# furkanyesiler/acoss

Hardware: AMD Instinct MI355X
Metric: track-pairs/sec on N x N Serra09 Qmax (HPCP, T=2000) (higher is better)
Workload: dtype f32

## Files before the change

### acoss_amd/_lib.py

```python
import ctypes
import os

import numpy as np

_HERE = os.path.dirname(os.path.abspath(__file__))
LIB_PATH = os.environ.get("ACX_LIB") or os.path.join(_HERE, "csrc", "libacx.so")

ACX_OK = 0
ACX_ERR_INVALID = -1
ACX_ERR_HIP = -2
ACX_ERR_NOMEM = -3
ACX_ERR_STATE = -4
ACX_ERR_SHORT = -5
ACX_ERR_UNSUPPORTED = -6

EXPORTS = [
    "acx_abi_version", "acx_create", "acx_destroy", "acx_last_error", "acx_set_scratch_limit",
    "acx_upload_pool", "acx_serra09_default_params", "acx_serra09_pairs", "acx_serra09_debug_pair",
    "acx_serra09_embed_len", "acx_profile_enable", "acx_profile_reset", "acx_profile_count",
    "acx_profile_get", "acx_debug_sqrt", "acx_debug_ef_sqrt", "acx_upload_pool_f64", "acx_simple_pairs",
    "acx_ef_upload_pool", "acx_earlyfusion_pairs", "acx_ef_debug_pair", "acx_sw_binary",
    "acx_chenfusion_pairs", "acx_csm_binary_sw", "acx_upload_raw_pool", "acx_download_pool",
    "acx_simple_upload_raw_pool", "acx_download_pool_f64", "acx_snf_fuse", "acx_qmax_binary",
    "acx_ef_block_features", "acx_ef_upload_raw_pool", "acx_snf_fuse_dists", "acx_grid_plan", "acx_pool_lengths", "acx_grid_run", "acx_grid_scatter", "acx_pair_grid",
    "acx_set_nonfinite_policy", "acx_nonfinite_zeroed", "acx_ef_pool_begin", "acx_ef_pool_tracks", "acx_ef_pool_end",
    "acx_set_ef_gemm", "acx_hip_versions",
    "acx_dev_alloc", "acx_dev_free", "acx_dev_read", "acx_dev_sync",
    "acx_comm_id", "acx_comm_init", "acx_comm_destroy", "acx_grid_allgather", "acx_pair_grid_ranks", "acx_set_ef_fuse",
    "acx_device_info", "acx_ef_debug_pairs",
    "acx_ftm2d_default_params", "acx_ftm2d_pool_begin", "acx_ftm2d_pool_tracks", "acx_ftm2d_pool_end",
    "acx_ftm2d_upload_shingles", "acx_ftm2d_download_shingles", "acx_ftm2d_debug_track", "acx_ftm2d_pairs",
    "acx_rank_columns", "acx_topk_rows",
    "acx_query_scores", "acx_query_topk", "acx_query_ranks", "acx_query_topk_lists",
    "acx_serra09_debug_bits", "acx_serra09_plan", "acx_serra09_family_name",
    "acx_pool_append", "acx_pool_append_raw", "acx_pool_append_f64", "acx_ef_pool_append", "acx_ftm2d_append_shingles",
    "acx_pool_truncate",
    "acx_serra09_align", "acx_qmax_locate_binary",
    "acx_serra09_align_paths", "acx_qmax_path_binary",
]
ABI_VERSION = 4
COMM_ID_BYTES = 128

ALGO_SERRA09, ALGO_CHENFUSION, ALGO_SIMPLE, ALGO_EARLYFUSION, ALGO_FTM2D = 0, 1, 2, 3, 4
GRID_PLANES = {ALGO_SERRA09: 1, ALGO_CHENFUSION: 2, ALGO_SIMPLE: 1, ALGO_EARLYFUSION: 4, ALGO_FTM2D: 1}


class AcxError(RuntimeError):
    """A libacx call failed (HIP error, missing device, out of device memory ...)."""

# ... 130 lines not shown
    L.acx_set_nonfinite_policy.argtypes = [vp, ctypes.c_int32]
    L.acx_nonfinite_zeroed.restype = ctypes.c_int64
    L.acx_nonfinite_zeroed.argtypes = [vp]
    L.acx_upload_pool.argtypes = [vp, fp, lp, ctypes.c_int32, ctypes.c_int32]
    L.acx_upload_raw_pool.argtypes = [vp, fp, lp, ctypes.c_int32, ctypes.c_int32, ctypes.c_int32, lp]
    L.acx_download_pool.argtypes = [vp, fp, ctypes.c_int64]
    L.acx_serra09_default_params.restype = None
    L.acx_serra09_default_params.argtypes = [pp]
    L.acx_serra09_pairs.argtypes = [vp, ip, ctypes.c_int64, pp, fp]
    L.acx_chenfusion_pairs.argtypes = [vp, ip, ctypes.c_int64, pp, fp]
    L.acx_serra09_debug_pair.argtypes = [vp, ctypes.c_int32, ctypes.c_int32, pp, fp, fp, fp, fp, fp, ip, fp, ip]
    L.acx_serra09_debug_bits.argtypes = [vp, ip, ctypes.c_int64, pp, fp, ctypes.POINTER(ctypes.c_uint8), ctypes.POINTER(ctypes.c_int64)]
    L.acx_serra09_plan.argtypes = [lp, ctypes.c_int32, ip, ctypes.c_int64, pp, ctypes.c_int64, ctypes.POINTER(Serra09PlanRec)]
    L.acx_serra09_family_name.restype = ctypes.c_char_p
    L.acx_serra09_family_name.argtypes = [ctypes.c_int32, ctypes.c_int32]
    L.acx_serra09_embed_len.restype = ctypes.c_int32
    L.acx_serra09_embed_len.argtypes = [ctypes.c_int32, pp]
    L.acx_profile_enable.argtypes = [vp, ctypes.c_int]
    L.acx_profile_reset.argtypes = [vp]
    L.acx_profile_count.argtypes = [vp]
    L.acx_profile_get.argtypes = [vp, ctypes.c_int, ctypes.c_char_p, ctypes.c_int,
                                  ctypes.POINTER(ctypes.c_double), lp, lp]
    L.acx_debug_sqrt.argtypes = [vp, fp, ctypes.c_int64, fp]
    L.acx_debug_ef_sqrt.argtypes = [vp, fp, ctypes.c_int64, fp]
    dp = ctypes.POINTER(ctypes.c_double)
    L.acx_upload_pool_f64.argtypes = [vp, dp, lp, ctypes.c_int32, ctypes.c_int32]
    L.acx_simple_upload_raw_pool.argtypes = [vp, fp, lp, ctypes.c_int32, ctypes.c_int32, ctypes.c_int32, ctypes.c_int32,
                                             ctypes.c_int32, lp]
    L.acx_download_pool_f64.argtypes = [vp, dp, ctypes.c_int64]
    L.acx_simple_pairs.argtypes = [vp, ip, ctypes.c_int64, ctypes.c_int32, ctypes.c_int32, dp]
# ... 144 lines not shown
def serra09_plan(lengths, pairs, params=None, scratch_limit=0):
    L = load()
    lengths = np.ascontiguousarray(lengths, dtype=np.int64)
    pairs = np.ascontiguousarray(pairs, dtype=np.int32).reshape(-1, 2)
    params = params if params is not None else serra09_params()
    out = np.zeros(len(pairs), dtype=np.dtype(Serra09PlanRec))
    rc = L.acx_serra09_plan(_lptr(lengths), len(lengths), _iptr(pairs), len(pairs), ctypes.byref(params), int(scratch_limit),
                            out.ctypes.data_as(ctypes.POINTER(Serra09PlanRec)))
    if rc != ACX_OK:
        err = AcxError("acx_serra09_plan: code %d: %s" % (rc, (L.acx_last_error(None) or b"bad argument").decode()))
        err.code = rc
        raise err
    return out


def serra09_family_name(family, m):
    name = load().acx_serra09_family_name(int(family), int(m))
    if name is None:
        raise ValueError("unknown Serra09 kernel family %r" % (family,))
    return name.decode()


def grid_scatter(lengths, spec, gathered, rank_stride, planes, mirror, first=0, count=-1):
    L = load()
    lengths = np.ascontiguousarray(lengths, dtype=np.int64)
    gathered = np.ascontiguousarray(gathered, dtype=np.float32)
    n = len(lengths)
    for P in planes:
        if P.dtype != np.float32 or P.shape != (n, n) or not P.flags["C_CONTIGUOUS"]:
            raise ValueError("grid_scatter: planes must be C-contiguous (N, N) float32")
# ... 726 lines not shown
```

### acoss_amd/csrc/acx.hip

```cpp
#include <hip/hip_runtime.h>

#include <chrono>
#include <dlfcn.h>
#include <rccl/rccl.h>

#include <algorithm>
#include <cmath>
#include <cstdio>
#include <cstdlib>
#include <cstring>
#include <string>
#include <vector>

#include "../../include/acx.h"
#include "serra09_kernels.hpp"
#include "serra09_long_kernels.hpp"
#include "serra09_locate_kernels.hpp"
#include "serra09_path_kernels.hpp"
#include "prep_kernels.hpp"
#include "snf_kernels.hpp"
#include "simple_kernels.hpp"
#include "ef_kernels.hpp"
#include "ef_rowstat2_kernels.hpp"
#include "ef_gemm_dma_kernels.hpp"
// ... 271 lines not shown
{
    if (p.m < 1 || p.m > acx::MAX_M_LONG) return fail(c, ACX_ERR_UNSUPPORTED, "serra09: m must be in 1..33 on the device");
    if (p.tau < 1) return fail(c, ACX_ERR_INVALID, "serra09: tau must be >= 1");
    if (!(p.kappa >= 0.0f && p.kappa <= 1.0f)) return fail(c, ACX_ERR_INVALID, "serra09: kappa must be in [0, 1]");
    if (p.dp_start != 2 && p.dp_start != 3) return fail(c, ACX_ERR_INVALID, "serra09: dp_start must be 2 or 3");
    if (p.pct_mode < 0 || p.pct_mode > 3) return fail(c, ACX_ERR_INVALID, "serra09: pct_mode must be 0..3");
    if (p.oti_target != 0 && p.oti_target != 1) return fail(c, ACX_ERR_INVALID, "serra09: oti_target must be 0 or 1");
    if (!(p.gamma_o >= 0.0f) || !(p.gamma_e >= 0.0f)) return fail(c, ACX_ERR_INVALID, "serra09: gammas must be >= 0");
    if (p.arith != ACX_ARITH_EXACT && p.arith != ACX_ARITH_F16X2) return fail(c, ACX_ERR_INVALID, "serra09: arith must be ACX_ARITH_EXACT or ACX_ARITH_F16X2");
    if (p.arith == ACX_ARITH_F16X2 && p.m != 9) return fail(c, ACX_ERR_UNSUPPORTED, "serra09: the f16x2 Gram exists for the default stack size m = 9 only");
    return ACX_OK;
}

constexpr int64_t POOL_SLACK = 96;

bool launch_band(acx_ctx *c, int m, const PairDesc *dpd, int B, int maxRows, int cls, const acx_serra09_params &p, int role, int write_d2,
                 int want_eps)
{
    const float *operands = p.arith == ACX_ARITH_F16X2 ? reinterpret_cast<const float *>(c->d_fh + POOL_SLACK * acx::FH) : c->d_frot + POOL_SLACK * acx::FROT;
    acx::BandLaunch L{c->stream, operands, c->active_toff(), c->d_normtab + POOL_SLACK, c->d_noff, c->d_scratch, c->d_thr,
                      c->d_bits, p.kappa, p.pct_mode, p.inclusive, p.oti_target};
    return acx::launch_band_kernel(L, m, dpd, B, maxRows, acx::serra09_band_family(cls, m, p.arith), role, write_d2, want_eps, p.arith);
}

template <int M>
void launch_normtab(acx_ctx *c, int maxM, int span, int first, int count)
{
    hipLaunchKernelGGL((acx::normtab_kernel<M>), dim3(count, (maxM + 255) / 256, acx::NBIN), dim3(256), 0, c->stream,
                       c->active_frames(), c->active_toff() + first, c->d_noff + first, c->d_normtab + POOL_SLACK, span);
}

#ifdef ACX_FAST_BUILD
#ifndef ACX_FAST_BUILD_M
#define ACX_FAST_BUILD_M 9
#endif
#define ACX_M_SWITCH(m_, CALL) switch (m_) { case ACX_FAST_BUILD_M: CALL(ACX_FAST_BUILD_M); break; default: handled = false; }
#else
// ... 477 lines not shown
        }
        int64_t cls_cells[NC + 1];
        for (int cl = 0; cl <= NC; ++cl) {
            cls_cells[cl] = 0;
            const int b0 = cls_begin[cl], Bc = cls_begin[cl + 1] - b0;
            if (Bc <= 0) continue;
            const acx::Serra09Extent ce = acx::serra09_extent(pd, b0, b0 + Bc);
            cls_cells[cl] = ce.cells;
            if (cl < NC) {
                bool ok = true;
                for (int cq = 0; cq < NC; ++cq) {
                    const int q0 = key_begin[NC * cl + cq], Bq = key_begin[NC * cl + cq + 1] - q0;
                    if (Bq <= 0) continue;
                    const acx::Serra09Extent qe = acx::serra09_extent(pd, q0, q0 + Bq);
                    ProfScope ps(c, KS_BAND, qe.cells);
                    ok = ok && launch_band(c, p.m, S.d_pd + q0, Bq, qe.Mr, cq, p, 1, 0, dbg ? 1 : 0);
                }
                if (!bits_free) { ACX_HIP(c, hipStreamWaitEvent(c->stream, Sprev.done, 0)); bits_free = true; }
                {
                    ProfScope ps(c, KS_BAND, ce.cells);
                    ok = ok && launch_band(c, p.m, S.d_pd + b0, Bc, ce.Mq, cl, p, 0, dbg ? 1 : 0, dbg ? 1 : 0);
                }
                if (use_q) ACX_HIP(c, hipEventRecord(S.cls_ev[cl], c->stream));
                if (!ok) return fail(c, ACX_ERR_UNSUPPORTED, "serra09: this build of libacx has no band kernel for the requested m");
            } else {
                if (!bits_free) { ACX_HIP(c, hipStreamWaitEvent(c->stream, Sprev.done, 0)); bits_free = true; }
                launch_streaming_class(c, S.d_pd + b0, &pd[b0], Bc, ce, p);
            }
        }
        {
            hipError_t wait_err = hipSuccess;
            auto sweep = [&](bool dmax, float *dst, hipStream_t qs) {
                for (int cl = 0; cl <= NC; ++cl) {
                    const int b0 = cls_begin[cl], Bc = cls_begin[cl + 1] - b0;
                    if (Bc <= 0) continue;
                    if (use_q) { const hipError_t e_ = hipStreamWaitEvent(qs, S.cls_ev[cl], 0); if (e_ != hipSuccess) wait_err = e_; }
// ... 2823 lines not shown
                r.Mq = pd[k2].Mq; r.Mr = pd[k2].Mr;
                r.batch = batch;
                r.cr = cl; r.cq = band ? acx::serra09_row_class(pd[k2].Mq) : acx::SERRA09_NC;
                r.row_family = band ? acx::serra09_band_family(r.cr, params->m, params->arith) : ACX_SERRA09_FAMILY_STREAMING;
                r.col_family = band ? acx::serra09_band_family(r.cq, params->m, params->arith) : ACX_SERRA09_FAMILY_STREAMING;
                r.sweep_cols = sw.cols; r.sweep_pack = sw.pack;
            }
        }
        k0 = k;
    }
    return ACX_OK;
}

const char *acx_serra09_family_name(int32_t family, int32_t m) { return acx::serra09_family_name(family, m); }

int acx_pool_lengths(acx_ctx *c, int32_t algo, int64_t *lengths, int32_t capacity, int32_t *n_tracks)
{
    if (!c) return ACX_ERR_INVALID;
    std::vector<int64_t> len;
    const int rc = pool_lengths(c, algo, len);
    if (rc != ACX_OK) return rc;
    if (n_tracks) *n_tracks = (int32_t)len.size();
    if (lengths) {
        if (capacity < (int32_t)len.size()) return fail(c, ACX_ERR_INVALID, "pool_lengths: buffer too small");
        std::copy(len.begin(), len.end(), lengths);
    }
    return ACX_OK;
}

static const std::vector<acx_grid_tile> &cached_plan(acx_ctx *c, const std::vector<int64_t> &len, const acx_grid_spec &spec)
// ... 996 lines not shown
```

### acoss_amd/csrc/acx_band.hip

```cpp
#include <hip/hip_runtime.h>

#include "serra09_kernels.hpp"
#include "serra09_band2_kernels.hpp"
#include "serra09_plan.hpp"

namespace acx {

namespace {

template <int M>
bool launch_band_m(const BandLaunch &L, const PairDesc *dpd, int B, int maxRows, int family, int role, int write_d2, int want_eps, int arith)
{
    const dim3 grid((maxRows + BAND - 1) / BAND, B, 1);
#define ACX_BAND_K(V4_, R_, W_, A_) hipLaunchKernelGGL((band_kernel<M, V4_, R_, W_, A_>), grid, dim3(BAND_THREADS), 0, L.stream, \
                                                  L.frot, L.toff, L.normtab, L.noff, dpd, L.scratch, L.thr, L.bits, L.kappa, \
                                                  L.pct_mode, L.inclusive, L.oti_target, want_eps)
#define ACX_BAND_A(V4_, A_) do { if (role) ACX_BAND_K(V4_, 1, false, A_); else if (write_d2) ACX_BAND_K(V4_, 0, true, A_); else ACX_BAND_K(V4_, 0, false, A_); } while (0)
#define ACX_BAND(V4_) do { if (arith == ACX_ARITH_EXACT) ACX_BAND_A(V4_, 0); else if constexpr (M == 9) ACX_BAND_A(V4_, 1); else return false; return true; } while (0)
#define ACX_BAND2_K(R_, W_, NV_, GL_) hipLaunchKernelGGL((band2_kernel<M, R_, W_, NV_, GL_>), grid, dim3(64 * B2Geom<NV_, GL_>::WAVES), 0, L.stream, L.frot, L.normtab, \
                                                         dpd, L.scratch, L.thr, L.bits, L.pct_mode, L.inclusive, L.oti_target, want_eps)
#define ACX_BAND2(NV_, GL_) do { if constexpr (M <= 9) { if (arith != ACX_ARITH_EXACT) return false; \
                                     if (role) ACX_BAND2_K(1, false, NV_, GL_); else if (write_d2) ACX_BAND2_K(0, true, NV_, GL_); else ACX_BAND2_K(0, false, NV_, GL_); \
                                     return true; } return false; } while (0)
    if (arith != ACX_ARITH_EXACT && arith != ACX_ARITH_F16X2) return false;
    switch (family) {
    case ACX_SERRA09_FAMILY_BAND2_4ROWS: ACX_BAND2(B2_NV, 16);
    case ACX_SERRA09_FAMILY_BAND2_2ROWS: ACX_BAND2(B2_NV, 32);
    case ACX_SERRA09_FAMILY_BAND2_MID: ACX_BAND2(B2_NV_MID, 32);
    case ACX_SERRA09_FAMILY_BAND_2: ACX_BAND(2);
    case ACX_SERRA09_FAMILY_BAND_4: ACX_BAND(4);
    case ACX_SERRA09_FAMILY_BAND_8: ACX_BAND(8);
    }
// ... 13 lines not shown
#define ACX_CASE(M_) case M_: return launch_band_m<M_>(L, dpd, B, maxRows, family, role, write_d2, want_eps, arith);
#ifdef ACX_FAST_BUILD
#ifndef ACX_FAST_BUILD_M
#define ACX_FAST_BUILD_M 9
#endif
        ACX_CASE(ACX_FAST_BUILD_M)
#else
        ACX_CASE(1) ACX_CASE(2) ACX_CASE(3) ACX_CASE(4) ACX_CASE(5) ACX_CASE(6) ACX_CASE(7) ACX_CASE(8)
        ACX_CASE(9) ACX_CASE(10) ACX_CASE(11) ACX_CASE(12) ACX_CASE(13) ACX_CASE(14) ACX_CASE(15) ACX_CASE(16)
#endif
#undef ACX_CASE
    }
    return false;
}


}

#ifdef ACX_TIMING
extern "C" int acx_dev_band_timing(unsigned long long *out, int reset)
{
    if (hipDeviceSynchronize() != hipSuccess) return -1;
    if (hipMemcpyFromSymbol(out, HIP_SYMBOL(acx::g_band_clk), sizeof(unsigned long long) * 32) != hipSuccess) return -1;
    if (reset) {
        unsigned long long z[32] = {0};
        if (hipMemcpyToSymbol(HIP_SYMBOL(acx::g_band_clk), z, sizeof(z)) != hipSuccess) return -1;
    }
    return 0;
}
#endif
// ... 1 lines not shown
```

### acoss_amd/csrc/serra09_kernels.hpp

```cpp
#pragma once
#include <hip/hip_runtime.h>
#include <stdint.h>
#include <type_traits>

namespace acx {

constexpr int NBIN = 12;
constexpr int SEL_BINS = 2048;
constexpr int MAX_M = 16;
constexpr int NGUARD = 80;

struct PctPos { float kf, fl, ce; int32_t ilo, ihi, k; };
__host__ __device__ inline PctPos pct_position(int n, float kappa, int pct_mode)
{
    PctPos p;
    p.kf = (n > 1) ? (float)(n - 1) * kappa : (float)n * kappa;
    p.fl = floorf(p.kf); p.ce = ceilf(p.kf);
    int ilo = (int)p.fl, ihi = (int)p.ce;
    ilo = ilo < 0 ? 0 : (ilo > n - 1 ? n - 1 : ilo);
    ihi = ihi < 0 ? 0 : (ihi > n - 1 ? n - 1 : ihi);
    int k = ilo;
    if (pct_mode == 3) {
        k = (int)floorf(p.kf + 0.5f);
        k = k > n - 1 ? n - 1 : k;
// ... 747 lines not shown
    if (e >= n) return;
    const int t = e / NBIN, b = e - t * NBIN;
    out[o0 * NBIN + e] = in[(toff_in[track] + (int64_t)t * tau) * NBIN + b];
}

struct BandLaunch {
    hipStream_t stream;
    const float *frot;
    const int64_t *toff;
    const float *normtab;
    const int64_t *noff;
    float *scratch, *thr;
    unsigned long long *bits;
    float kappa;
    int pct_mode, inclusive, oti_target;
};
bool launch_band_kernel(const BandLaunch &L, int m, const struct PairDesc *dpd, int B, int maxRows, int family, int role,
                        int write_d2, int want_eps, int arith);

#ifdef ACX_ABL
#define ACX_ABL_EXIT(n_, val_) do { if (ACX_ABL == (n_)) { if ((val_) == 1.2345e-30f) thr[0] = 1.0f; return; } } while (0)
#else
#define ACX_ABL_EXIT(n_, val_) do { } while (0)
#endif

#ifdef ACX_TIMING
__device__ unsigned long long g_band_clk[32];
struct StampT { unsigned long long t; int base; };
#define ACX_STAMP(slot) do { const unsigned long long now_ = __builtin_readcyclecounter(); \
        if (lane == 0) atomicAdd(&g_band_clk[tstamp_.base + (slot)], now_ - tstamp_.t); tstamp_.t = now_; } while (0)
#else
#define ACX_STAMP(slot) do { } while (0)
#endif
// ... 36 lines not shown
    static constexpr bool HIST_IN_ROW = ROWP >= 64 + 2 * FBINS;
    static constexpr int PBINS = NV >= 32 ? 512 : 256;
    static constexpr int PGRP = NV >= 32 ? 1 : 2;
    static constexpr float PDELTA = NV >= 32 ? 0.04f : (NV >= 16 ? 0.15f : 0.0f);
    static constexpr int GBINS = 32 * NV;
    static constexpr int TAIL_FLOATS = BAND * ROWP + (HIST_IN_ROW ? 0 : 8 * FBINS);
    static_assert(SelGeom<GBINS>::SLOTS + 64 + 4 <= ROWP, "generic selection must fit the wave's own exchange row");
    static_assert(HIST_IN_ROW || (BAND * ROWP) % FBINS == 0, "fast histograms must be aligned to their size");
    static_assert(NV == 8 || NV == 16 || NV == 32, "row owners hold 8, 16 or 32 consecutive slots");
    __device__ static __forceinline__ int hist_off(int wave)
    {
        return HIST_IN_ROW ? ((wave * ROWP + 64 + FBINS - 1) & ~(FBINS - 1)) : BAND * ROWP + wave * FBINS;
    }
};

template <int NV, int ROLE, bool TC_VIA_LDS, typename TCG>
__device__ __forceinline__ void band_row_bits(const float (&xr)[NV], const TCG (&tcg)[NV / 4], float thr_row, float *myrow, int lane,
                                              int row, int MB, int cshift, const PairDesc &P, float *__restrict__ thr,
                                              unsigned long long *__restrict__ bits)
{
    using RG = RowGeom<NV>;
    constexpr int CH = NV / 4;
    typedef float f32x4_u __attribute__((ext_vector_type(4), aligned(4)));
    float *X = thr + P.offX;
    if (ROLE == 0 && bits) {
        float tcv[NV];
        if constexpr (TC_VIA_LDS) {
            float *tr = myrow + 4 * lane + 4 * ((4 * lane) / NV);
#pragma unroll
            for (int q = 0; q < CH; ++q) *reinterpret_cast<float4 *>(tr + q * (256 + 4 * (256 / NV))) = make_float4(tcg[q].x, tcg[q].y, tcg[q].z, tcg[q].w);
            wave_lds_fence();
            const float *mine = myrow + lane * RG::LNP;
#pragma unroll
            for (int j = 0; j < CH; ++j) {
                const float4 v = *reinterpret_cast<const float4 *>(mine + 4 * j);
                tcv[4 * j + 0] = v.x; tcv[4 * j + 1] = v.y; tcv[4 * j + 2] = v.z; tcv[4 * j + 3] = v.w;
            }
        } else {
            const float *tc = X + P.pitchT + (lane * NV - cshift);
#pragma unroll
            for (int j = 0; j < CH; ++j) {
                const f32x4_u v = *reinterpret_cast<const f32x4_u *>(tc + 4 * j);
                tcv[4 * j + 0] = v.x; tcv[4 * j + 1] = v.y; tcv[4 * j + 2] = v.z; tcv[4 * j + 3] = v.w;
            }
        }
        int lo = cshift - lane * NV, hi = MB + cshift - lane * NV;
        lo = lo < 0 ? 0 : lo;
        hi = hi > NV ? NV : hi;
        unsigned valid = 0u;
        if (hi > lo) valid = (hi - lo >= 32 ? ~0u : ((1u << (hi - lo)) - 1u)) << lo;
        unsigned acc = 0u;
#pragma unroll
        for (int t = NV - 1; t >= 0; --t) {
            float mthr;
            asm("v_min_f32 %0, %1, %2" : "=v"(mthr) : "v"(tcv[t]), "v"(thr_row));
            asm("v_cmp_le_f32 vcc, %1, %2\n\tv_addc_co_u32 %0, vcc, %0, %0, vcc" : "+v"(acc) : "v"(xr[t]), "v"(mthr) : "vcc");
        }
        acc &= valid;
        if constexpr (NV == 16) {
            acc |= (unsigned)__builtin_amdgcn_update_dpp(0, (int)acc, 0xF5, 0xf, 0xf, false) << 16;
        } else if constexpr (NV == 8) {
            acc |= (unsigned)__builtin_amdgcn_update_dpp(0, (int)acc, 0xF9, 0xf, 0xf, false) << 8;
            acc |= (unsigned)__builtin_amdgcn_update_dpp(0, (int)acc, 0xFE, 0xf, 0xf, false) << 16;
        }
        constexpr int LPD = 32 / NV;
        unsigned *rowbits = reinterpret_cast<unsigned *>(bits + P.offT + (size_t)row * P.nw);
        const int ndw = 2 * P.nw, d = lane / LPD;
        if ((lane & (LPD - 1)) == 0 && d < ndw) rowbits[d] = acc;
        for (int z = 2 * NV + lane; z < ndw; z += 64) rowbits[z] = 0u;
    }
}

#ifdef ACX_TIMING
#define ACX_STAMP_PARM , StampT &tstamp_
#define ACX_STAMP_ARG , tstamp_
#else
#define ACX_STAMP_PARM
#define ACX_STAMP_ARG
#endif
template <int NV, int ROLE, bool SNAP = true>
__device__ __forceinline__ void band_row_tail(float (&xr)[NV], float *smem, int wave, int lane, int row, int MA, int MB,
                                              int cshift, const PairDesc &P, float *__restrict__ thr,
                                              unsigned long long *__restrict__ bits, const PctPos &pp, int pct_mode,
                                              int inclusive, int want_eps ACX_STAMP_PARM)
{
    using RG = RowGeom<NV>;
    constexpr int ROWP = RG::ROWP, FBINS = RG::FBINS, FCOPIES = RG::FCOPIES, PBINS = RG::PBINS, PGRP = RG::PGRP, GBINS = RG::GBINS;
    constexpr bool HIST_IN_ROW = RG::HIST_IN_ROW;
    constexpr float PDELTA = RG::PDELTA;
    constexpr int CH = NV / 4;
    constexpr int role = ROLE;
    const float INF = __builtin_inff();
    const int hist_off = RG::hist_off(wave);
    if (row >= MA) return;
    const int n = MB;
    const float kf = pp.kf, fl = pp.fl, ce = pp.ce;
    const int ilo = pp.ilo, ihi = pp.ihi, k = pp.k;
    const bool interp = (pct_mode == 0 || pct_mode == 1);
    float *myrow = smem + wave * ROWP;
    float slo, shi;
    typedef __attribute__((address_space(3))) void lds_void;
    const unsigned hist_addr = (unsigned)(uintptr_t)(lds_void *)(smem + hist_off);
    const bool use_pivot = (ihi + 2) * 9 <= n;
    auto zero_hist = [&](int bins) {
        float *h = smem + hist_off;
        for (int q = 0; q < bins / 256; ++q) *reinterpret_cast<float4 *>(h + 256 * q + 4 * lane) = make_float4(0.f, 0.f, 0.f, 0.f);
        wave_lds_fence();
    };
    if constexpr (HIST_IN_ROW) zero_hist(use_pivot ? PBINS : FBINS);
    bool done = false;
    const int end_valid = MB + cshift;
    const bool lane_has_data = lane * NV < end_valid;
    if (use_pivot) {
        const int g0 = (lane & ~(PGRP - 1)) * NV;
        const bool group_full = g0 >= cshift && g0 + PGRP * NV <= end_valid;
        done = wave_select_pivot<NV, PBINS, PGRP>(xr, k, interp && ihi != ilo, hist_addr, myrow, lane, slo, shi,
                                                  lane_has_data, group_full, PDELTA);
        if (!done) zero_hist(FBINS);
    }
    if (!done)
        done = wave_select_fast<NV, FBINS, FCOPIES>(xr, k, interp && ihi != ilo, hist_addr, myrow, lane, slo, shi, lane_has_data);
    if (!done) {
        unsigned *ghist = reinterpret_cast<unsigned *>(myrow) + 64;
        unsigned *counter = reinterpret_cast<unsigned *>(myrow) + 64 + SelGeom<GBINS>::SLOTS;
        const SelectResult sr = wave_select_regs<NV, GBINS>(xr, k, ghist, myrow, counter, lane, interp);
        slo = sr.value;
        shi = (interp && ihi != ilo && sr.cnt_le <= ihi) ? sr.next : sr.value;
    }
    ACX_STAMP(5);
    ACX_ABL_EXIT(3, slo + shi);
    typedef float f32x4_u __attribute__((ext_vector_type(4), aligned(4)));
    constexpr bool TC_VIA_LDS = NV >= 32;
    f32x4_u tcg[CH];
    if constexpr (TC_VIA_LDS) {
        if (role == 0 && bits) {
            asm volatile("" ::: "memory");
            const float *tc = thr + P.offX + P.pitchT - cshift + 4 * lane;
#pragma unroll
            for (int q = 0; q < CH; ++q) tcg[q] = *reinterpret_cast<const f32x4_u *>(tc + 256 * q);
        }
    }
    const bool weights_ok = interp && ihi == ilo + 1 && inclusive && fl >= 1.0f && (ce - kf) >= 0.00390625f && (kf - fl) >= 0.00390625f;
    if (SNAP && !want_eps && weights_ok && shi < INF && (shi - slo) > shi * 0.000244140625f) {
        ACX_STAMP(6);
        ACX_ABL_EXIT(4, slo);
        if (lane == 0) (thr + P.offX)[role ? P.pitchT + row : row] = slo;
        band_row_bits<NV, ROLE, TC_VIA_LDS>(xr, tcg, slo, myrow, lane, row, MB, cshift, P, thr, bits);
        ACX_STAMP(7);
        return;
    }
    float dlo, dhi;
    const float eps = percentile_eps2(slo, shi, pct_mode, ilo, ihi, kf, fl, ce, dlo, dhi);
    float thr_row;
    if (SNAP && inclusive && dlo <= eps && eps < dhi) thr_row = slo;
    else thr_row = d2_threshold(eps, inclusive);
    ACX_STAMP(6);
    float *X = thr + P.offX;
    if (lane == 0) {
        const int o = role ? P.pitchT + row : row;
        X[o] = thr_row;
        X[P.pitchT + P.pitchD + o] = eps;
    }
    band_row_bits<NV, ROLE, TC_VIA_LDS>(xr, tcg, thr_row, myrow, lane, row, MB, cshift, P, thr, bits);
    ACX_STAMP(7);
}

constexpr int band_waves_per_simd(int m, int v4, int arith = 0) { return (v4 <= 2 && m <= 9) ? ACX_NARROW_WAVES : ((v4 <= 4 && m <= 9) ? (arith ? 6 : ACX_MID_WAVES) : 4); }
template <int M, int V4, int ROLE, bool WD2 = false, int ARITH = 0>
__global__ __launch_bounds__(BAND_THREADS, band_waves_per_simd(M, V4, ARITH)) void band_kernel(const float *__restrict__ frot,
                                                            const int64_t *__restrict__ toff,
                                                            const float *__restrict__ normtab,
                                                            const int64_t *__restrict__ noff,
                                                            const PairDesc *__restrict__ pd,
                                                            float *__restrict__ scratch,
                                                            float *__restrict__ thr,
                                                            unsigned long long *__restrict__ bits,
                                                            float kappa, int pct_mode, int inclusive, int oti_target, int want_eps)
{
    constexpr bool write_d2 = WD2;
    using G = BandGeom<M, V4, ARITH>;
    constexpr int role = ROLE;
    constexpr int NV = 4 * V4;
    constexpr int NSTEP = NV / 8;
    using RG = RowGeom<NV>;
    constexpr int LNP = RG::LNP, ROWP = RG::ROWP, FBINS = RG::FBINS;
    constexpr bool HIST_IN_ROW = RG::HIST_IN_ROW;
    constexpr int SWEEP_FLOATS = 8 * G::AROWS * G::SP;
    constexpr int LDS_FLOATS = SWEEP_FLOATS > RG::TAIL_FLOATS ? SWEEP_FLOATS : RG::TAIL_FLOATS;
    __shared__ __attribute__((aligned(4096))) float smem[LDS_FLOATS];

    const int bid_x = blockIdx.x, bid_y = blockIdx.y;
    const PairDesc P = pd[bid_y];
    const int MA = role ? P.Mr : P.Mq, MB = role ? P.Mq : P.Mr;
    const int TA = role ? P.Tr : P.Tq, TB = role ? P.Tq : P.Tr;
// ... 266 lines not shown
        const float *mine = smem + wave * ROWP + lane * LNP;
#pragma unroll
        for (int j = 0; j < CH; ++j) {
            const float4 v = *reinterpret_cast<const float4 *>(mine + 4 * j);
            xr[4 * j + 0] = v.x; xr[4 * j + 1] = v.y; xr[4 * j + 2] = v.z; xr[4 * j + 3] = v.w;
        }
    }

    asm volatile("s_waitcnt lgkmcnt(0)" ::: "memory");
    ACX_STAMP(4);
#ifdef ACX_ABL
    { float keep_ = 0.0f;
      for (int t = 0; t < NV; ++t) keep_ += xr[t];
      ACX_ABL_EXIT(2, keep_); }
#endif
    band_row_tail<NV, ROLE, ARITH == 0 || ROLE == 0>(xr, smem, wave, lane, i0 + wave, MA, MB, (BAND - 1) - wave, P, thr, role == 0 ? bits : nullptr,
                            pp, pct_mode, inclusive, want_eps ACX_STAMP_ARG);
}

template <bool EQG, bool DMAX, int CPL>
__device__ __forceinline__ void qmax_cells(unsigned wraw, unsigned colmask, unsigned wprev, unsigned wleft,
                                           float l1a, float l1b, float l2a, float p1a, float p1b, float p2a,
                                           const float (&QA)[CPL], float (&QB)[CPL],
                                           const float (&PA)[EQG ? 1 : CPL], float (&PB)[EQG ? 1 : CPL],
                                           float go, float ge, float &best)
{
    const unsigned w = wraw & colmask;
#pragma unroll
    for (int e = CPL - 1; e >= 0; --e) {
        const bool r = (w >> e) & 1u;
        float x3 = 0.0f, x4 = 0.0f;
// ... 342 lines not shown
```

### acoss_amd/csrc/serra09_plan.hpp

```cpp
#pragma once
#include <algorithm>
#include <cstdint>
#include <cstdlib>
#include <vector>

#include "../../include/acx.h"
#include "serra09_kernels.hpp"

namespace acx {

inline int serra09_tiles(int M) { return (M + BAND - 1 + 63) / 64; }

inline int64_t serra09_round_up(int64_t v, int64_t m) { return (v + m - 1) / m * m; }

inline int serra09_embed_len(int T, int m, int tau, int embed_full)
{
    const int span = embed_full ? (m - 1) * tau : m * tau;
    const int L = T - span;
    if (L <= 0) return 0;
    return (L + tau - 1) / tau;
}

constexpr int SERRA09_NC = 5;
struct Serra09Class {
// ... 169 lines not shown
    for (int kk = 0; kk < SERRA09_NKEY; ++kk) s.key_begin[kk + 1] = s.key_begin[kk] + fill[kk];
    for (int kk = 0; kk < SERRA09_NKEY; ++kk) fill[kk] = s.key_begin[kk];
    perm.resize(B);
    tmp.resize(B);
    for (int k2 = 0; k2 < B; ++k2) {
        const int kk = serra09_pair_key(pd[k2], m);
        perm[fill[kk]] = k2;
        tmp[fill[kk]++] = pd[k2];
    }
    pd.swap(tmp);
    for (int cl = 0; cl <= SERRA09_NC; ++cl) s.cls_begin[cl] = s.key_begin[SERRA09_NC * cl];
    s.cls_begin[SERRA09_NC + 1] = B;
    return s;
}

struct Serra09Extent { int Mq = 0, Mr = 0; int64_t cells = 0; };
inline Serra09Extent serra09_extent(const std::vector<PairDesc> &pd, int b0, int b1)
{
    Serra09Extent e;
    for (int k2 = b0; k2 < b1; ++k2) {
        e.Mq = std::max(e.Mq, pd[k2].Mq); e.Mr = std::max(e.Mr, pd[k2].Mr);
        e.cells += (int64_t)pd[k2].Mq * pd[k2].Mr;
    }
    return e;
}

}
```

### include/acx.h

```cpp
#ifndef ACX_H
#define ACX_H

#include <stdint.h>

#ifdef __cplusplus
extern "C" {
#endif

#define ACX_ABI_VERSION 4

enum {
    ACX_OK = 0,
    ACX_ERR_INVALID = -1,
    ACX_ERR_HIP = -2,
    ACX_ERR_NOMEM = -3,
    ACX_ERR_STATE = -4,
    ACX_ERR_SHORT = -5,
    ACX_ERR_UNSUPPORTED = -6
};

typedef struct acx_ctx acx_ctx;


acx_ctx *acx_create(int device, int *err);
// ... 79 lines not shown
    ACX_SERRA09_FAMILY_BAND_2 = 3,
    ACX_SERRA09_FAMILY_BAND_4 = 4,
    ACX_SERRA09_FAMILY_BAND_8 = 5,
    ACX_SERRA09_FAMILY_STREAMING = 6
};
typedef struct acx_serra09_plan_rec {
    int32_t Mq, Mr;
    int32_t batch;
    int32_t cr, cq;
    int32_t row_family, col_family;
    int32_t sweep_cols, sweep_pack;
} acx_serra09_plan_rec;
int acx_serra09_plan(const int64_t *lengths, int32_t n_tracks, const int32_t *pairs, int64_t K,
                     const acx_serra09_params *params, int64_t scratch_limit, acx_serra09_plan_rec *out);
const char *acx_serra09_family_name(int32_t family, int32_t m);


int acx_upload_pool_f64(acx_ctx *ctx, const double *frames, const int64_t *offsets,
                        int32_t n_tracks, int32_t dim);

int acx_simple_upload_raw_pool(acx_ctx *ctx, const float *raw, const int64_t *raw_offsets, int32_t n_tracks,
                               int32_t dim, int32_t win, int32_t skip, int32_t win_len_smooth,
                               int64_t *pooled_offsets_out);

int acx_download_pool_f64(acx_ctx *ctx, double *frames, int64_t capacity);

int acx_simple_pairs(acx_ctx *ctx, const int32_t *pairs, int64_t K, int32_t sslen, int32_t oti,
                     double *out);


// ... 187 lines not shown
```

Measured before the change: 106,000.

## Add specialized fast-tail band kernel for wide exact-arithmetic rows

Adds a compile-time FAST variant of the band kernel's row tail. When the host can show that a run of pairs meets the interpolation, pivot and snap conditions, the variant fixes pct_mode, inclusive and eps, drops the validity masking and the zero-fill of trailing bit words, and hints the easy branches as likely. The host splits each band launch into runs of fast and regular pairs and issues a separate launch per run. This adds template instantiations and possibly more launches, and it relies on the host-side checks exactly matching the device conditions, since the mask and zero-fill are skipped.

```diff
diff --git a/acoss_amd/_lib.py b/acoss_amd/_lib.py
--- a/acoss_amd/_lib.py
+++ b/acoss_amd/_lib.py
@@ -32,7 +32,7 @@
     "acx_ftm2d_upload_shingles", "acx_ftm2d_download_shingles", "acx_ftm2d_debug_track", "acx_ftm2d_pairs",
     "acx_rank_columns", "acx_topk_rows",
     "acx_query_scores", "acx_query_topk", "acx_query_ranks", "acx_query_topk_lists",
-    "acx_serra09_debug_bits", "acx_serra09_plan", "acx_serra09_family_name",
+    "acx_serra09_debug_bits", "acx_serra09_plan", "acx_serra09_family_name", "acx_serra09_fast_tail", "acx_serra09_fast_tail_launches",
     "acx_pool_append", "acx_pool_append_raw", "acx_pool_append_f64", "acx_ef_pool_append", "acx_ftm2d_append_shingles",
     "acx_pool_truncate",
     "acx_serra09_align", "acx_qmax_locate_binary",
@@ -193,6 +193,9 @@
     L.acx_serra09_plan.argtypes = [lp, ctypes.c_int32, ip, ctypes.c_int64, pp, ctypes.c_int64, ctypes.POINTER(Serra09PlanRec)]
     L.acx_serra09_family_name.restype = ctypes.c_char_p
     L.acx_serra09_family_name.argtypes = [ctypes.c_int32, ctypes.c_int32]
+    L.acx_serra09_fast_tail.argtypes = [pp, ctypes.c_int32, ctypes.c_int32, ctypes.c_int32]
+    L.acx_serra09_fast_tail_launches.restype = ctypes.c_int64
+    L.acx_serra09_fast_tail_launches.argtypes = []
     L.acx_serra09_embed_len.restype = ctypes.c_int32
     L.acx_serra09_embed_len.argtypes = [ctypes.c_int32, pp]
     L.acx_profile_enable.argtypes = [vp, ctypes.c_int]
@@ -367,6 +370,19 @@
     return out
 
 
+def serra09_fast_tail(n_cells, role, params=None, debug=False):
+    L = load()
+    params = params if params is not None else serra09_params()
+    rc = L.acx_serra09_fast_tail(ctypes.byref(params), int(n_cells), int(role), int(bool(debug)))
+    if rc < 0:
+        raise ValueError("acx_serra09_fast_tail: bad argument")
+    return bool(rc)
+
+
+def serra09_fast_tail_launches():
+    return int(load().acx_serra09_fast_tail_launches())
+
+
 def serra09_family_name(family, m):
     name = load().acx_serra09_family_name(int(family), int(m))
     if name is None:
diff --git a/acoss_amd/csrc/acx.hip b/acoss_amd/csrc/acx.hip
--- a/acoss_amd/csrc/acx.hip
+++ b/acoss_amd/csrc/acx.hip
@@ -309,13 +309,19 @@
 
 constexpr int64_t POOL_SLACK = 96;
 
-bool launch_band(acx_ctx *c, int m, const PairDesc *dpd, int B, int maxRows, int cls, const acx_serra09_params &p, int role, int write_d2,
-                 int want_eps)
+bool launch_band(acx_ctx *c, int m, const PairDesc *dpd, const std::vector<PairDesc> &hpd, int b0, int B, int maxRows, int cls,
+                 const acx_serra09_params &p, int role, int write_d2, int want_eps)
 {
     const float *operands = p.arith == ACX_ARITH_F16X2 ? reinterpret_cast<const float *>(c->d_fh + POOL_SLACK * acx::FH) : c->d_frot + POOL_SLACK * acx::FROT;
     acx::BandLaunch L{c->stream, operands, c->active_toff(), c->d_normtab + POOL_SLACK, c->d_noff, c->d_scratch, c->d_thr,
-                      c->d_bits, p.kappa, p.pct_mode, p.inclusive, p.oti_target};
-    return acx::launch_band_kernel(L, m, dpd, B, maxRows, acx::serra09_band_family(cls, m, p.arith), role, write_d2, want_eps, p.arith);
+                      c->d_bits, p.kappa, p.pct_mode, p.inclusive, p.oti_target, 0};
+    const int family = acx::serra09_band_family(cls, m, p.arith);
+    bool ok = true;
+    for (const acx::Serra09Run &r : acx::serra09_fast_tail_runs(p, family, role, write_d2 != 0, want_eps != 0, c->d_bits != nullptr, hpd, b0, b0 + B)) {
+        L.fast_tail = r.fast ? 1 : 0;
+        ok = ok && acx::launch_band_kernel(L, m, dpd + (r.begin - b0), r.end - r.begin, maxRows, family, role, write_d2, want_eps, p.arith);
+    }
+    return ok;
 }
 
 template <int M>
@@ -823,12 +829,12 @@
                     if (Bq <= 0) continue;
                     const acx::Serra09Extent qe = acx::serra09_extent(pd, q0, q0 + Bq);
                     ProfScope ps(c, KS_BAND, qe.cells);
-                    ok = ok && launch_band(c, p.m, S.d_pd + q0, Bq, qe.Mr, cq, p, 1, 0, dbg ? 1 : 0);
+                    ok = ok && launch_band(c, p.m, S.d_pd + q0, pd, q0, Bq, qe.Mr, cq, p, 1, 0, dbg ? 1 : 0);
                 }
                 if (!bits_free) { ACX_HIP(c, hipStreamWaitEvent(c->stream, Sprev.done, 0)); bits_free = true; }
                 {
                     ProfScope ps(c, KS_BAND, ce.cells);
-                    ok = ok && launch_band(c, p.m, S.d_pd + b0, Bc, ce.Mq, cl, p, 0, dbg ? 1 : 0, dbg ? 1 : 0);
+                    ok = ok && launch_band(c, p.m, S.d_pd + b0, pd, b0, Bc, ce.Mq, cl, p, 0, dbg ? 1 : 0, dbg ? 1 : 0);
                 }
                 if (use_q) ACX_HIP(c, hipEventRecord(S.cls_ev[cl], c->stream));
                 if (!ok) return fail(c, ACX_ERR_UNSUPPORTED, "serra09: this build of libacx has no band kernel for the requested m");
@@ -3682,6 +3688,18 @@
 
 const char *acx_serra09_family_name(int32_t family, int32_t m) { return acx::serra09_family_name(family, m); }
 
+int64_t acx_serra09_fast_tail_launches(void) { return (int64_t)acx::fast_tail_launches(); }
+
+int acx_serra09_fast_tail(const acx_serra09_params *params, int32_t n_cells, int32_t role, int32_t debug)
+{
+    if (!params || n_cells < 1 || check_params(nullptr, *params) != ACX_OK) return ACX_ERR_INVALID;
+    const int cl = acx::serra09_row_class(n_cells);
+    if (cl >= acx::SERRA09_NC || params->m > acx::MAX_M) return 0;
+    const bool dbg = debug != 0;
+    return acx::serra09_fast_tail_params(*params, acx::serra09_band_family(cl, params->m, params->arith), role, dbg && role == 0, dbg, true) &&
+           acx::serra09_fast_tail_row(acx::pct_position(n_cells, params->kappa, params->pct_mode), n_cells) ? 1 : 0;
+}
+
 int acx_pool_lengths(acx_ctx *c, int32_t algo, int64_t *lengths, int32_t capacity, int32_t *n_tracks)
 {
     if (!c) return ACX_ERR_INVALID;
diff --git a/acoss_amd/csrc/acx_band.hip b/acoss_amd/csrc/acx_band.hip
--- a/acoss_amd/csrc/acx_band.hip
+++ b/acoss_amd/csrc/acx_band.hip
@@ -1,4 +1,7 @@
 #include <hip/hip_runtime.h>
+
+#include <atomic>
+#include <cassert>
 
 #include "serra09_kernels.hpp"
 #include "serra09_band2_kernels.hpp"
@@ -8,14 +11,22 @@
 
 namespace {
 
+std::atomic<long long> g_fast_tail_launches{0};
+
 template <int M>
 bool launch_band_m(const BandLaunch &L, const PairDesc *dpd, int B, int maxRows, int family, int role, int write_d2, int want_eps, int arith)
 {
     const dim3 grid((maxRows + BAND - 1) / BAND, B, 1);
-#define ACX_BAND_K(V4_, R_, W_, A_) hipLaunchKernelGGL((band_kernel<M, V4_, R_, W_, A_>), grid, dim3(BAND_THREADS), 0, L.stream, \
+#define ACX_BAND_K(V4_, R_, W_, A_, F_) hipLaunchKernelGGL((band_kernel<M, V4_, R_, W_, A_, F_>), grid, dim3(BAND_THREADS), 0, L.stream, \
                                                   L.frot, L.toff, L.normtab, L.noff, dpd, L.scratch, L.thr, L.bits, L.kappa, \
                                                   L.pct_mode, L.inclusive, L.oti_target, want_eps)
-#define ACX_BAND_A(V4_, A_) do { if (role) ACX_BAND_K(V4_, 1, false, A_); else if (write_d2) ACX_BAND_K(V4_, 0, true, A_); else ACX_BAND_K(V4_, 0, false, A_); } while (0)
+#define ACX_BAND_A(V4_, A_) do { if (role) ACX_BAND_K(V4_, 1, false, A_, false); else if (write_d2) ACX_BAND_K(V4_, 0, true, A_, false); else ACX_BAND_K(V4_, 0, false, A_, false); } while (0)
+    if (L.fast_tail) {
+        assert(family == ACX_SERRA09_FAMILY_BAND_8 && arith == ACX_ARITH_EXACT && !write_d2 && !want_eps);
+        if (role) ACX_BAND_K(8, 1, false, 0, true); else ACX_BAND_K(8, 0, false, 0, true);
+        g_fast_tail_launches.fetch_add(1, std::memory_order_relaxed);
+        return true;
+    }
 #define ACX_BAND(V4_) do { if (arith == ACX_ARITH_EXACT) ACX_BAND_A(V4_, 0); else if constexpr (M == 9) ACX_BAND_A(V4_, 1); else return false; return true; } while (0)
 #define ACX_BAND2_K(R_, W_, NV_, GL_) hipLaunchKernelGGL((band2_kernel<M, R_, W_, NV_, GL_>), grid, dim3(64 * B2Geom<NV_, GL_>::WAVES), 0, L.stream, L.frot, L.normtab, \
                                                          dpd, L.scratch, L.thr, L.bits, L.pct_mode, L.inclusive, L.oti_target, want_eps)
@@ -59,6 +70,7 @@
     return false;
 }
 
+long long fast_tail_launches() { return g_fast_tail_launches.load(std::memory_order_relaxed); }
 
 }
 
diff --git a/acoss_amd/csrc/serra09_kernels.hpp b/acoss_amd/csrc/serra09_kernels.hpp
--- a/acoss_amd/csrc/serra09_kernels.hpp
+++ b/acoss_amd/csrc/serra09_kernels.hpp
@@ -785,9 +785,11 @@
     unsigned long long *bits;
     float kappa;
     int pct_mode, inclusive, oti_target;
+    int fast_tail;
 };
 bool launch_band_kernel(const BandLaunch &L, int m, const struct PairDesc *dpd, int B, int maxRows, int family, int role,
                         int write_d2, int want_eps, int arith);
+long long fast_tail_launches();
 
 #ifdef ACX_ABL
 #define ACX_ABL_EXIT(n_, val_) do { if (ACX_ABL == (n_)) { if ((val_) == 1.2345e-30f) thr[0] = 1.0f; return; } } while (0)
@@ -854,7 +856,7 @@
     }
 };
 
-template <int NV, int ROLE, bool TC_VIA_LDS, typename TCG>
+template <int NV, int ROLE, bool TC_VIA_LDS, bool FAST = false, bool MASK = true, typename TCG>
 __device__ __forceinline__ void band_row_bits(const float (&xr)[NV], const TCG (&tcg)[NV / 4], float thr_row, float *myrow, int lane,
                                               int row, int MB, int cshift, const PairDesc &P, float *__restrict__ thr,
                                               unsigned long long *__restrict__ bits)
@@ -863,7 +865,7 @@
     constexpr int CH = NV / 4;
     typedef float f32x4_u __attribute__((ext_vector_type(4), aligned(4)));
     float *X = thr + P.offX;
-    if (ROLE == 0 && bits) {
+    if (ROLE == 0 && (FAST || bits)) {
         float tcv[NV];
         if constexpr (TC_VIA_LDS) {
             float *tr = myrow + 4 * lane + 4 * ((4 * lane) / NV);
@@ -884,11 +886,13 @@
                 tcv[4 * j + 0] = v.x; tcv[4 * j + 1] = v.y; tcv[4 * j + 2] = v.z; tcv[4 * j + 3] = v.w;
             }
         }
-        int lo = cshift - lane * NV, hi = MB + cshift - lane * NV;
-        lo = lo < 0 ? 0 : lo;
-        hi = hi > NV ? NV : hi;
         unsigned valid = 0u;
-        if (hi > lo) valid = (hi - lo >= 32 ? ~0u : ((1u << (hi - lo)) - 1u)) << lo;
+        if constexpr (MASK) {
+            int lo = cshift - lane * NV, hi = MB + cshift - lane * NV;
+            lo = lo < 0 ? 0 : lo;
+            hi = hi > NV ? NV : hi;
+            if (hi > lo) valid = (hi - lo >= 32 ? ~0u : ((1u << (hi - lo)) - 1u)) << lo;
+        }
         unsigned acc = 0u;
 #pragma unroll
         for (int t = NV - 1; t >= 0; --t) {
@@ -896,7 +900,7 @@
             asm("v_min_f32 %0, %1, %2" : "=v"(mthr) : "v"(tcv[t]), "v"(thr_row));
             asm("v_cmp_le_f32 vcc, %1, %2\n\tv_addc_co_u32 %0, vcc, %0, %0, vcc" : "+v"(acc) : "v"(xr[t]), "v"(mthr) : "vcc");
         }
-        acc &= valid;
+        if constexpr (MASK) acc &= valid;
         if constexpr (NV == 16) {
             acc |= (unsigned)__builtin_amdgcn_update_dpp(0, (int)acc, 0xF5, 0xf, 0xf, false) << 16;
         } else if constexpr (NV == 8) {
@@ -907,7 +911,8 @@
         unsigned *rowbits = reinterpret_cast<unsigned *>(bits + P.offT + (size_t)row * P.nw);
         const int ndw = 2 * P.nw, d = lane / LPD;
         if ((lane & (LPD - 1)) == 0 && d < ndw) rowbits[d] = acc;
-        for (int z = 2 * NV + lane; z < ndw; z += 64) rowbits[z] = 0u;
+        if constexpr (!(FAST && NV == 32))
+            for (int z = 2 * NV + lane; z < ndw; z += 64) rowbits[z] = 0u;
     }
 }
 
@@ -918,7 +923,7 @@
 #define ACX_STAMP_PARM
 #define ACX_STAMP_ARG
 #endif
-template <int NV, int ROLE, bool SNAP = true>
+template <int NV, int ROLE, bool SNAP = true, bool FAST = false>
 __device__ __forceinline__ void band_row_tail(float (&xr)[NV], float *smem, int wave, int lane, int row, int MA, int MB,
                                               int cshift, const PairDesc &P, float *__restrict__ thr,
                                               unsigned long long *__restrict__ bits, const PctPos &pp, int pct_mode,
@@ -932,16 +937,18 @@
     constexpr int role = ROLE;
     const float INF = __builtin_inff();
     const int hist_off = RG::hist_off(wave);
+    static_assert(!FAST || SNAP, "the product-path tail snaps its thresholds");
     if (row >= MA) return;
     const int n = MB;
     const float kf = pp.kf, fl = pp.fl, ce = pp.ce;
     const int ilo = pp.ilo, ihi = pp.ihi, k = pp.k;
-    const bool interp = (pct_mode == 0 || pct_mode == 1);
+    if constexpr (FAST) { pct_mode = 0; inclusive = 1; want_eps = 0; }
+    const bool interp = FAST || (pct_mode == 0 || pct_mode == 1);
     float *myrow = smem + wave * ROWP;
     float slo, shi;
     typedef __attribute__((address_space(3))) void lds_void;
     const unsigned hist_addr = (unsigned)(uintptr_t)(lds_void *)(smem + hist_off);
-    const bool use_pivot = (ihi + 2) * 9 <= n;
+    const bool use_pivot = FAST || (ihi + 2) * 9 <= n;
     auto zero_hist = [&](int bins) {
         float *h = smem + hist_off;
         for (int q = 0; q < bins / 256; ++q) *reinterpret_cast<float4 *>(h + 256 * q + 4 * lane) = make_float4(0.f, 0.f, 0.f, 0.f);
@@ -954,18 +961,19 @@
     if (use_pivot) {
         const int g0 = (lane & ~(PGRP - 1)) * NV;
         const bool group_full = g0 >= cshift && g0 + PGRP * NV <= end_valid;
-        done = wave_select_pivot<NV, PBINS, PGRP>(xr, k, interp && ihi != ilo, hist_addr, myrow, lane, slo, shi,
+        done = wave_select_pivot<NV, PBINS, PGRP>(xr, k, FAST || (interp && ihi != ilo), hist_addr, myrow, lane, slo, shi,
                                                   lane_has_data, group_full, PDELTA);
+        if constexpr (FAST) done = __builtin_expect(done, true);
         if (!done) zero_hist(FBINS);
     }
     if (!done)
-        done = wave_select_fast<NV, FBINS, FCOPIES>(xr, k, interp && ihi != ilo, hist_addr, myrow, lane, slo, shi, lane_has_data);
+        done = wave_select_fast<NV, FBINS, FCOPIES>(xr, k, FAST || (interp && ihi != ilo), hist_addr, myrow, lane, slo, shi, lane_has_data);
     if (!done) {
         unsigned *ghist = reinterpret_cast<unsigned *>(myrow) + 64;
         unsigned *counter = reinterpret_cast<unsigned *>(myrow) + 64 + SelGeom<GBINS>::SLOTS;
         const SelectResult sr = wave_select_regs<NV, GBINS>(xr, k, ghist, myrow, counter, lane, interp);
         slo = sr.value;
-        shi = (interp && ihi != ilo && sr.cnt_le <= ihi) ? sr.next : sr.value;
+        shi = ((FAST || (interp && ihi != ilo)) && sr.cnt_le <= ihi) ? sr.next : sr.value;
     }
     ACX_STAMP(5);
     ACX_ABL_EXIT(3, slo + shi);
@@ -973,19 +981,21 @@
     constexpr bool TC_VIA_LDS = NV >= 32;
     f32x4_u tcg[CH];
     if constexpr (TC_VIA_LDS) {
-        if (role == 0 && bits) {
+        if (role == 0 && (FAST || bits)) {
             asm volatile("" ::: "memory");
             const float *tc = thr + P.offX + P.pitchT - cshift + 4 * lane;
 #pragma unroll
             for (int q = 0; q < CH; ++q) tcg[q] = *reinterpret_cast<const f32x4_u *>(tc + 256 * q);
         }
     }
-    const bool weights_ok = interp && ihi == ilo + 1 && inclusive && fl >= 1.0f && (ce - kf) >= 0.00390625f && (kf - fl) >= 0.00390625f;
-    if (SNAP && !want_eps && weights_ok && shi < INF && (shi - slo) > shi * 0.000244140625f) {
+    const bool weights_ok = FAST || (interp && ihi == ilo + 1 && inclusive && fl >= 1.0f && (ce - kf) >= 0.00390625f && (kf - fl) >= 0.00390625f);
+    bool easy = SNAP && !want_eps && weights_ok && shi < INF && (shi - slo) > shi * 0.000244140625f;
+    if constexpr (FAST) easy = __builtin_expect(easy, true);
+    if (easy) {
         ACX_STAMP(6);
         ACX_ABL_EXIT(4, slo);
         if (lane == 0) (thr + P.offX)[role ? P.pitchT + row : row] = slo;
-        band_row_bits<NV, ROLE, TC_VIA_LDS>(xr, tcg, slo, myrow, lane, row, MB, cshift, P, thr, bits);
+        band_row_bits<NV, ROLE, TC_VIA_LDS, FAST, !FAST>(xr, tcg, slo, myrow, lane, row, MB, cshift, P, thr, bits);
         ACX_STAMP(7);
         return;
     }
@@ -1001,12 +1011,12 @@
         X[o] = thr_row;
         X[P.pitchT + P.pitchD + o] = eps;
     }
-    band_row_bits<NV, ROLE, TC_VIA_LDS>(xr, tcg, thr_row, myrow, lane, row, MB, cshift, P, thr, bits);
+    band_row_bits<NV, ROLE, TC_VIA_LDS, FAST>(xr, tcg, thr_row, myrow, lane, row, MB, cshift, P, thr, bits);
     ACX_STAMP(7);
 }
 
 constexpr int band_waves_per_simd(int m, int v4, int arith = 0) { return (v4 <= 2 && m <= 9) ? ACX_NARROW_WAVES : ((v4 <= 4 && m <= 9) ? (arith ? 6 : ACX_MID_WAVES) : 4); }
-template <int M, int V4, int ROLE, bool WD2 = false, int ARITH = 0>
+template <int M, int V4, int ROLE, bool WD2 = false, int ARITH = 0, bool FAST = false>
 __global__ __launch_bounds__(BAND_THREADS, band_waves_per_simd(M, V4, ARITH)) void band_kernel(const float *__restrict__ frot,
                                                             const int64_t *__restrict__ toff,
                                                             const float *__restrict__ normtab,
@@ -1018,6 +1028,7 @@
                                                             float kappa, int pct_mode, int inclusive, int oti_target, int want_eps)
 {
     constexpr bool write_d2 = WD2;
+    static_assert(!FAST || (V4 == 8 && ARITH == 0 && !WD2), "the product-path tail exists for the wide class of the exact arithmetic");
     using G = BandGeom<M, V4, ARITH>;
     constexpr int role = ROLE;
     constexpr int NV = 4 * V4;
@@ -1314,7 +1325,7 @@
       for (int t = 0; t < NV; ++t) keep_ += xr[t];
       ACX_ABL_EXIT(2, keep_); }
 #endif
-    band_row_tail<NV, ROLE, ARITH == 0 || ROLE == 0>(xr, smem, wave, lane, i0 + wave, MA, MB, (BAND - 1) - wave, P, thr, role == 0 ? bits : nullptr,
+    band_row_tail<NV, ROLE, ARITH == 0 || ROLE == 0, FAST>(xr, smem, wave, lane, i0 + wave, MA, MB, (BAND - 1) - wave, P, thr, role == 0 ? bits : nullptr,
                             pp, pct_mode, inclusive, want_eps ACX_STAMP_ARG);
 }
 
diff --git a/acoss_amd/csrc/serra09_plan.hpp b/acoss_amd/csrc/serra09_plan.hpp
--- a/acoss_amd/csrc/serra09_plan.hpp
+++ b/acoss_amd/csrc/serra09_plan.hpp
@@ -207,6 +207,32 @@
     return s;
 }
 
+inline bool serra09_fast_tail_row(const PctPos &pp, int n)
+{
+    return pp.ihi == pp.ilo + 1 && pp.fl >= 1.0f && (pp.ce - pp.kf) >= 0.00390625f && (pp.kf - pp.fl) >= 0.00390625f && (pp.ihi + 2) * 9 <= n;
+}
+inline bool serra09_fast_tail_params(const acx_serra09_params &p, int family, int role, bool write_d2, bool want_eps, bool have_bits)
+{
+    return family == ACX_SERRA09_FAMILY_BAND_8 && p.arith == ACX_ARITH_EXACT && p.pct_mode == 0 && p.inclusive != 0 && !write_d2 && !want_eps &&
+           (role != 0 || have_bits);
+}
+struct Serra09Run { int begin, end; bool fast; };
+inline std::vector<Serra09Run> serra09_fast_tail_runs(const acx_serra09_params &p, int family, int role, bool write_d2, bool want_eps,
+                                                       bool have_bits, const std::vector<PairDesc> &pd, int b0, int b1)
+{
+    std::vector<Serra09Run> runs;
+    if (b1 <= b0) return runs;
+    if (!serra09_fast_tail_params(p, family, role, write_d2, want_eps, have_bits)) return {Serra09Run{b0, b1, false}};
+    auto ok = [&](int k2) { return role ? serra09_fast_tail_row(pd[k2].pos_q, pd[k2].Mq) : serra09_fast_tail_row(pd[k2].pos_r, pd[k2].Mr); };
+    for (int k2 = b0; k2 < b1; ++k2) {
+        const bool f = ok(k2);
+        if (!runs.empty() && runs.back().fast == f) runs.back().end = k2 + 1;
+        else runs.push_back(Serra09Run{k2, k2 + 1, f});
+    }
+    if ((int)runs.size() > 2 + (b1 - b0) / 32) return {Serra09Run{b0, b1, false}};
+    return runs;
+}
+
 struct Serra09Extent { int Mq = 0, Mr = 0; int64_t cells = 0; };
 inline Serra09Extent serra09_extent(const std::vector<PairDesc> &pd, int b0, int b1)
 {
diff --git a/include/acx.h b/include/acx.h
--- a/include/acx.h
+++ b/include/acx.h
@@ -117,6 +117,8 @@
 int acx_serra09_plan(const int64_t *lengths, int32_t n_tracks, const int32_t *pairs, int64_t K,
                      const acx_serra09_params *params, int64_t scratch_limit, acx_serra09_plan_rec *out);
 const char *acx_serra09_family_name(int32_t family, int32_t m);
+int acx_serra09_fast_tail(const acx_serra09_params *params, int32_t n_cells, int32_t role, int32_t debug);
+int64_t acx_serra09_fast_tail_launches(void);
 
 
 int acx_upload_pool_f64(acx_ctx *ctx, const double *frames, const int64_t *offsets,
```

New measurement: 109,400 (median of 6 runs). 1.03x the previous value.
